# kngwyu/rogue-gym

Hardware: AMD Instinct MI355X
Metric: env-steps/sec (whole node) at 65 536 envs, 32x16 mini-dungeon (higher is better)
Workload: dtype u8/u16 integer state, f32 observation; 1 GPU; config-mini.json 32x16, 65536 envs per GPU (65536 total), gray-image obs [N,1,16,32] f32, max_steps 1000, auto-reset; envs_per_gpu=65536, parallelism=env-sharded x1, no data-path collective

## Files before the change

### rogue-gym_amd/csrc/rg_api.cpp

```cpp
#include <hip/hip_runtime.h>
#include <dlfcn.h>

#include <cstdio>
#include <cstdlib>
#include <cstring>
#include <mutex>
#include <random>
#include <string>
#include <vector>

#include "../../include/rogue_gym_hip.h"
#include "rg_state.h"
#include "rg_state_io.h"

extern "C" {
typedef struct ncclComm *ncclComm_t;
typedef struct { char internal[128]; } ncclUniqueId;
typedef int ncclResult_t;
typedef int ncclDataType_t;
}
static const ncclResult_t ncclSuccess = 0;
static const ncclDataType_t ncclUint8 = 1;

extern "C" {
// ... 2 lines not shown
void rgk_probe_clock(unsigned long long *out, int spin, hipStream_t st);
void rgk_regen(const RgState *SP, const RgConfig *c, int bulk, int spares, const uint32_t *mark, uint32_t target, uint32_t *err_any, hipStream_t st, hipEvent_t ev0, hipEvent_t ev1);
void rgk_regen_gate(const uint32_t *mark, uint32_t target, uint32_t *err_any, hipStream_t st);
void rgk_export(const RgState *S, uint32_t *err_any, void *o_screen, void *o_hist, void *o_status, void *o_flags, uint32_t *o_err, hipStream_t st);
int rgk_regen_lanes_supported(const RgConfig *c, int maze_cap);
int rgk_step_bound_capable(const RgConfig *c);
int rgk_regen_lanes(const RgState *SP, const RgConfig *c, uint32_t *q, int32_t *list, int bulk, int waves, int slots, hipStream_t st, hipEvent_t ev0, hipEvent_t ev1);
void rgk_debug_descend(const RgState *S, const RgConfig *c, hipStream_t st);
void rgk_render(const RgState *S, const RgConfig *c, hipStream_t st);
void rgk_encode(const uint8_t *screen, const uint8_t *hist, const int32_t *status, uint32_t *flags, uint32_t *err_any, int n, int hw, size_t rs, size_t rst,
                int symbols, int planes_sym, uint32_t sflag, int with_hist, int kind, float *out, const int32_t *ext, hipStream_t st);
void rgk_pack(const RgState *S, int with_hist, uint8_t *out, hipStream_t st);
void rgk_scatter_rows(const void *src, void *dst, const int32_t *ext, int n, int row_bytes, hipStream_t st);
void rgk_gather_keys(const uint8_t *keys, const int32_t *ext, uint8_t *dst, int n, hipStream_t st);
int rgk_obs(const RgState *S, const RgConfig *c, uint32_t sflag, int with_hist, int kind, float *out, uint32_t *err_any, int planes_sym, int bound, hipStream_t st, hipEvent_t ev0, hipEvent_t ev1);
int rgk_redraw(const RgState *S, const RgConfig *c, hipStream_t st);
int rgk_obs_typed(const RgState *S, const RgConfig *c, int kind, int dtype, uint32_t sflag, int with_hist, int planes_sym, void *out, uint32_t *err_any, hipStream_t st, hipEvent_t ev0,
                  hipEvent_t ev1);
int rgk_obs_crop(const RgState *S, const RgConfig *c, int kind, int ry, int rx, uint32_t sflag, int with_hist, int planes_sym, float *out, int32_t *centers,
                 uint32_t *err_any, hipStream_t st);
void rgk_state_save(const RgState *S, const RgIoLayout *L, const uint64_t *desc, const uint32_t *guard, const int32_t *ids, int k, uint8_t *out, hipStream_t st);
void rgk_state_load(const RgState *S, const RgIoLayout *L, const uint64_t *desc, const uint32_t *guard, const int32_t *ids, int k, const uint8_t *recs, uint32_t rec_bytes, uint8_t *ok,
                    uint8_t *mark, hipStream_t st);
}

#define RG_TIMED_KERNELS 5
struct rg_handle {
    RgParsed parsed;
    RgConfig cfg;
    RgState S;
// ... 5 lines not shown
    int lane_flip = 0;
    uint64_t lane_last = 0;
    uint8_t *pin_keys = nullptr;
    uint32_t *pin_err = nullptr;
    bool lane_regen = false;
    uint64_t step_count = 0;
    hipStream_t side = nullptr;
    int regen_idle_after = -1;
    int regen_bulk = 0;
    int device = 0;
    hipStream_t stream = nullptr;
    std::vector<void *> allocs;
    uint32_t *d_err = nullptr;
    uint8_t *d_keys = nullptr;
    bool render_pending = false;
    float *bound_out = nullptr; int bound_kind = 0; bool bound_valid = false;
    int32_t *obs_list_mem = nullptr; uint32_t *obs_cnt_mem = nullptr; float *gray_lut_mem = nullptr;
    int bound_steps = 0;
    int stair_gen = 0;
    float *obs_scratch = nullptr;
    size_t obs_scratch_cap = 0;
    std::vector<uint64_t> seed_lo, seed_hi;
    std::vector<uint8_t> reseed;
    std::vector<uint64_t> range_lo, range_span;
    unsigned long long *d_probe = nullptr;
    std::vector<rg_handle *> sub;
    std::vector<int> g_of, l_of;
    int32_t *d_ext = nullptr;
    std::vector<int32_t> ext;
    uint8_t *d_keys_sub = nullptr;
// ... 207 lines not shown
             dev_alloc(h, &P.p_exp, ns) && dev_alloc(h, &P.food, ns) && dev_alloc(h, &P.quiet, ns) && dev_alloc(h, &P.pack_gold, ns) && dev_alloc(h, &P.dlevel, ns) &&
             dev_alloc(h, &P.rng, 12 * ns) && dev_alloc(h, &P.room_rect, nr * ns) && dev_alloc(h, &P.room_meta, nr * ns) &&
             dev_alloc(h, &P.mon_w0, nr * ns) && dev_alloc(h, &P.mon_hp, nr * ns) && dev_alloc(h, &P.mon_exp, nr * ns) &&
             dev_alloc(h, &P.mon_cnt, ns) && dev_alloc(h, &P.gold_pos, nr * ns) && dev_alloc(h, &P.gold_amt, nr * ns) &&
             dev_alloc(h, &P.edge_a, ne * n) && dev_alloc(h, &P.edge_b, ne * n) && dev_alloc(h, &P.maze_stack, (size_t)maze_cap * n) &&
             dev_alloc(h, &P.on_stairs, ns);
        P.prof = nullptr;
        int lo = 0, hi = 0;
        if (ok && (hipDeviceGetStreamPriorityRange(&lo, &hi) != hipSuccess || hipStreamCreateWithPriority(&h->side, hipStreamNonBlocking, RG_DEV_ENV("ROGUE_GYM_HIP_SIDE_HIPRIO") ? hi : lo) != hipSuccess)) {
            h->err = "failed to create the background generation stream"; ok = false;
        }
        static const bool lanes_low = RG_DEV_ENV("ROGUE_GYM_HIP_LANES_LOWPRIO") != nullptr;
        if (ok && (hipStreamCreateWithPriority(&h->side2, hipStreamNonBlocking, lanes_low ? lo : (lo + hi) / 2) != hipSuccess || hipStreamCreateWithPriority(&h->side3, hipStreamNonBlocking, lanes_low ? lo : (lo + hi) / 2) != hipSuccess)) { h->err = "failed to create the background generation stream"; ok = false; }
    }
    ok = ok && dev_alloc(h, &h->d_SP, 1) && hipMemcpy(h->d_SP, &h->SP, sizeof(RgState), hipMemcpyHostToDevice) == hipSuccess;
    if (!ok) { g_create_err = h->err.empty() ? "device allocation failed" : h->err; destroy_handle(h); return 1; }
    if (hipMemset(S.screen, ' ', n * hw) != hipSuccess) { g_create_err = "hipMemset failed"; destroy_handle(h); return 1; }
    if (upload_seeds(h, n)) { g_create_err = h->err; destroy_handle(h); return 1; }
    h->S.stair_gen = h->stair_gen++;
    rgk_build(&h->S, &h->cfg, h->stream);
    hipError_t e = hipGetLastError();
    if (e == hipSuccess) e = hipStreamSynchronize(h->stream);
    if (e != hipSuccess) { g_create_err = std::string("k_build: ") + hipGetErrorString(e); destroy_handle(h); return 1; }
    h->render_pending = true;
    if (h->spares) {
        if (h->lane_regen && !(dev_alloc(h, &h->lane_q, 8) && dev_alloc(h, &h->lane_list, 2 * ns))) { g_create_err = h->err; destroy_handle(h); return 1; }
        if (h->lane_regen) (void)rgk_regen_lanes(&h->SP, &h->cfg, h->lane_q, h->lane_list, 1, 0, h->S.sp_slots, h->side2, nullptr, nullptr);
        else rgk_regen(&h->SP, &h->cfg, 1, 1, nullptr, 0, h->d_err, h->side, nullptr, nullptr);
        e = hipGetLastError();
        if (e == hipSuccess && !RG_DEV_ENV("ROGUE_GYM_HIP_ASYNC_FIRST_SPARES")) { e = hipStreamSynchronize(h->side); if (e == hipSuccess) e = hipStreamSynchronize(h->side2); if (e == hipSuccess) e = hipStreamSynchronize(h->side3); }
// ... 191 lines not shown
    if (!h->sub.empty()) {
        for (rg_handle *sh : h->sub) SUBCHK(h, sh, rg_reset(sh));
        h->screens_stale = true;
        return assemble_small(h);
    }
    h->S.stair_gen = h->stair_gen++;
    { TimedLaunch t(h, 3); rgk_build(&h->S, &h->cfg, h->stream); }
    HIPCHK(h, hipGetLastError());
    h->render_pending = true;
    h->bound_valid = false;
    return 0;
}

static int obs_common(rg_t *h, uint32_t status_flag, int with_hist, int kind, float *out_dev);
int rg_step(rg_t *h, const uint8_t *keys, int keys_on_device) { return rg_step_prefix(h, keys, h->S.n, keys_on_device); }
int rg_step_obs_gray(rg_t *h, const uint8_t *keys, int keys_on_device, uint32_t status_flag, int with_hist, float *out_dev) {
    return rg_step_prefix(h, keys, h->S.n, keys_on_device) ? 1 : obs_common(h, status_flag, with_hist, 0, out_dev);
}

int rg_step_prefix(rg_t *h, const uint8_t *keys, int n_keys, int keys_on_device) {
    HIPCHK(h, hipSetDevice(h->device));
    if (n_keys < 0) { h->err = "rg_step_prefix: negative key count"; return 1; }
    if (n_keys > h->S.n) n_keys = h->S.n;
    if (!h->sub.empty()) {
        const uint8_t *dkeys = keys;
        if (!keys_on_device) {
            if (!h->d_keys && !dev_alloc(h, &h->d_keys, (size_t)h->S.n)) return 1;
            HIPCHK(h, hipMemcpyAsync(h->d_keys, keys, (size_t)n_keys, hipMemcpyHostToDevice, h->stream));
            dkeys = h->d_keys;
        }
        for (rg_handle *sh : h->sub) {
            int m = 0;
            while (m < sh->S.n && sh->ext[m] < n_keys) m++;
            if (m) rgk_gather_keys(dkeys, sh->d_ext, sh->d_keys_sub, m, h->stream);
            SUBCHK(h, sh, rg_step_prefix(sh, sh->d_keys_sub, m, 1));
        }
        HIPCHK(h, hipGetLastError());
        h->screens_stale = true;
        return assemble_small(h);
    }
    if (flush_render(h)) return 1;
    const uint8_t *dk = keys;
    if (!keys_on_device) {
        HIPCHK(h, hipMemcpyAsync(h->d_keys, keys, (size_t)n_keys, hipMemcpyHostToDevice, h->stream));
        dk = h->d_keys;
    }
    h->S.n_keys = n_keys;
    static const int regen_every = RG_DEV_ENV("ROGUE_GYM_HIP_REGEN_EVERY") ? atoi(RG_DEV_ENV("ROGUE_GYM_HIP_REGEN_EVERY")) : 1;
    h->step_count++;
    bool regen = h->spares && (regen_every <= 1 || h->step_count % (uint64_t)regen_every == 0);
    if (regen && h->regen_idle_after >= 0) { if (h->regen_idle_after == 0) regen = false; else h->regen_idle_after--; }
    static const bool no_stair_waves = getenv("ROGUE_GYM_HIP_NO_STAIR_WAVES") != nullptr;
    {
        TimedLaunch t(h, 0, true);
        h->S.stair_gen = h->stair_gen++;
        h->S.obs_par = (int32_t)(h->step_count & 1); h->bound_steps++;
        (void)rgk_step(&h->S, h->d_SP, &h->cfg, dk, h->spares ? 1 : 0, no_stair_waves ? -1 : 0, h->stream, t.start_ev(), t.stop_ev());
    }
    HIPCHK(h, hipGetLastError());
    if (regen) {
        TimedLaunch t(h, 4, true);
        if (h->lane_regen) {
            static const int lane_waves = RG_DEV_ENV("ROGUE_GYM_HIP_LANE_WAVES") ? atoi(RG_DEV_ENV("ROGUE_GYM_HIP_LANE_WAVES")) : 256;
            static const int lane_every = RG_DEV_ENV("ROGUE_GYM_HIP_LANE_EVERY") ? atoi(RG_DEV_ENV("ROGUE_GYM_HIP_LANE_EVERY")) : 16;
            static const bool time_lanes = RG_DEV_ENV("ROGUE_GYM_HIP_TIME_LANES") != nullptr;
            const bool lanes_now = h->regen_bulk > 0 || h->step_count - h->lane_last >= (uint64_t)(lane_every > 0 ? lane_every : 1);
            static const int urgent_mode = RG_DEV_ENV("ROGUE_GYM_HIP_URGENT_AT0") ? 3 : 2;
            rgk_regen(&h->SP, &h->cfg, 0, urgent_mode, h->S.launch_mark, (uint32_t)h->S.stair_gen + 1u, h->d_err, h->side, time_lanes ? nullptr : t.start_ev(), time_lanes ? nullptr : t.stop_ev());
            if (time_lanes && !lanes_now) t.cancel();
            if (lanes_now) {
                h->lane_last = h->step_count;
                h->lane_flip ^= 1;
// ... 56 lines not shown
    HIPCHK(h, hipSetDevice(h->device));
    if (!h->sub.empty()) {
        for (rg_handle *sh : h->sub) {
            if (kind && sh->cfg.symbols > h->planes_sym) {
                h->err = "symbol image: a config of the batch has more symbols (" + std::to_string(sh->cfg.symbols) + ") than env 0's (" + std::to_string(h->planes_sym) +
                         "), which sets the channel count (python/src/lib.rs:281-285)";
                return 1;
            }
            SUBCHK(h, sh, obs_common(sh, status_flag, with_hist, kind, out_dev));
        }
        return 0;
    }
    {
        TimedLaunch t(h, 2, true);
        const bool bound = h->bound_out && out_dev == h->bound_out && kind == h->bound_kind && (status_flag & 0x1ffu) == 0 && !with_hist;
        if (rgk_obs(&h->S, &h->cfg, status_flag & 0x1ffu, with_hist ? 1 : 0, kind, out_dev, h->d_err, h->planes_sym, bound && h->S.obs_list && h->bound_valid && h->bound_steps == 1, h->stream, t.start_ev(), t.stop_ev())) {
            HIPCHK(h, hipGetLastError());
            h->render_pending = false;
            h->bound_valid = bound;
            h->bound_steps = 0;
            return 0;
        }
        t.cancel();
    }
    h->bound_valid = false;
    if (flush_render(h)) return 1;
    {
        TimedLaunch t(h, 2);
        rgk_encode(h->S.screen, h->S.hist, h->S.status, h->S.flags, h->d_err, h->S.n, h->S.hw, (size_t)h->S.hw, 10, h->cfg.symbols, h->planes_sym,
                   status_flag & 0x1ffu, with_hist ? 1 : 0, kind, out_dev, h->S.ext, h->stream);
    }
    HIPCHK(h, hipGetLastError());
// ... 846 lines not shown
```

### rogue-gym_amd/csrc/rg_kernels.hip

```cpp


#include "rg_device.h"


#include "rg_gen.h"


#ifdef RG_FINE_PROF
#define PFM(id) pf.mark(id)
#else
#define PFM(id) ((void)0)
#endif
struct Prof {
    unsigned long long *p; unsigned long long t, t0, r0; int k;
    __device__ __forceinline__ void start(unsigned long long *pp) { p = pp ? pp + (size_t)blockIdx.x * 64 : nullptr; k = 0; if (p) { r0 = __builtin_amdgcn_s_memrealtime(); t = t0 = __builtin_amdgcn_s_memtime(); } }
    __device__ __forceinline__ void rec(int phase, unsigned long long v) {
        if (p && threadIdx.x == 0 && k < 61) p[1 + k++] = ((unsigned long long)phase << 48) | (v & 0xffffffffffffull);
    }
    __device__ __forceinline__ void mark(int phase) {
        if (!p) return;
        unsigned long long now = __builtin_amdgcn_s_memtime();
        rec(phase, now - t);
        t = now;
    }
// ... 2088 lines not shown
#pragma nounroll
    for (int s0 = 0; s0 < nrooms; s0++)
        if ((actp >> (3 * s0)) & 2u) {
            const uint32_t m = mc[s0 * WAVE];
            const int x = POS_X(m), y = POS_Y(m);
            const uint32_t under = base_glyph(c, WV(w, WIN_K(x - w.ox, y - w.oy)), y);
            if ((under & 0x80u) && under != (0x80u | '*')) put(y * W + x, mt[(m >> 16) & 0xff]);
        }
    if (pl_moved && (base_glyph(c, WV(w, WIN_K(px - w.ox, py - w.oy)), py) & 0x80u)) put(py * W + px, '@');
    return true;
}

__device__ __forceinline__ void take_spares(const RgState &S, const RgState *__restrict__ SPd, const RgConfig &c, int lane, int e, bool taken, bool &on_stairs) {
    const uint64_t tm = __ballot(taken);
    if (!tm) return;
    const RgState &SP = *SPd;
    const int HW = S.hw, n = S.n, nrooms = c.room_num_x * c.room_num_y;
    const size_t ns = (size_t)n * S.sp_slots;
    int es = e;
    if (taken)
        for (int sl = S.sp_slots - 1; sl >= 0; sl--)
            if (__hip_atomic_load(&S.sp_ready[(size_t)sl * n + e], __ATOMIC_RELAXED, __HIP_MEMORY_SCOPE_AGENT) == 1u) es = sl * n + e;
    __builtin_amdgcn_fence(__ATOMIC_ACQUIRE, "agent");
    if ((HW & 7) == 0) {
        const int q = HW / 8;
        uint64_t mm = tm;
        while (mm) {
            const int s0 = __ffsll((long long)mm) - 1; mm &= mm - 1;
            const int s1 = mm ? __ffsll((long long)mm) - 1 : -1; if (mm) mm &= mm - 1;
            const int s2 = mm ? __ffsll((long long)mm) - 1 : -1; if (mm) mm &= mm - 1;
// ... 180 lines not shown
        uint64_t lag = __ballot(descends && ((old_flags & RG_FLAG_HIST_LAG) || ((old_flags & RG_FLAG_REDRAW) && (old_flags & RG_FLAG_HIST_STALE))));
        while (lag) {
            const int src = __ffsll((long long)lag) - 1;
            lag &= lag - 1;
            const int env_s = __shfl(e, src);
            const uint16_t *cp = S.cell + (size_t)env_s * S.hw;
            uint8_t *hp = S.hist + (size_t)env_s * S.hw;
            for (int i = lane; i < S.hw; i += WAVE) hp[i] = (cp[i] & C_VISITED) ? 1 : 0;
        }
    }
#pragma nounroll
    for (int pass = 0; pass < 2; ++pass) {
        pf.mark(1);
        if (pass == 1 && use_spares) {
            if (need_gen) {
                bool rdy = false;
                for (int sl = 0; sl < S.sp_slots; sl++) rdy = rdy || __hip_atomic_load(&S.sp_ready[(size_t)sl * S.n + e], __ATOMIC_RELAXED, __HIP_MEMORY_SCOPE_AGENT) == 1u;
                if (rdy) { taken = true; need_gen = false; n_taken++; }
            }
        }
        const bool regenerated = descends && pass == 0;
        if constexpr (BW == 1 || BW == 2) { if (pass == 0 && S.dc_walk) snapshot_walk_service(S, c, lane, e, descends); }
        const uint64_t nx_now = pass == 0 ? __ballot(need_gen && nxs == RG_NX_HIT) : 0ull;
        if (need_gen) n_inline++;
        gen_service<GM>(S, c, E, lane, e, need_gen, pass == 1, lds_grid, pf, nx_now);
        (void)regenerated;
        pf.mark(2);
        need_gen = false;
        if (pass == 1) break;

        bool running = live && act != ACT_NOOP;
        int iter = 0;
        while (__any(running)) {
// ... 116 lines not shown
    if (valid && err) {
        S.flags[et] = (old_flags & ~RG_FLAG_ERR_MASK) | err;
        S.reward[et] = 0.f;
        S.done[et] = (old_flags & RG_FLAG_TERMINAL) ? 1 : 0;
        atomicOr(S.err_any, err);
    } else if (valid && !live) {
        S.reward[et] = 0.f; S.done[et] = (old_flags & RG_FLAG_TERMINAL) ? 1 : 0;
    } else if (valid) {
        if (terminal && c.auto_reset) {
            if (taken) {
                E.dlevel = 1; E.gold = c.init_gold; E.hp = E.hpmax = c.init_hp; E.plvl = 1; E.exp = 0; E.food = c.hunger_time;
            }
            write_status(S, c, E);
            S.dc_len[et] = 0; S.dc_head[et] = 0; S.dc_part[et] = 0; S.dc_own[et] = 0;
            steps = 0;
            flags = RG_FLAG_REDRAW | RG_FLAG_HIST_DIRTY;
            klog_new_episode(S, et);
        }
        if (E.err) { flags |= E.err; atomicOr(S.err_any, E.err); }
        if (terminal) flags |= RG_FLAG_TERMINAL;
        if (!taken) store_env(S, E);
        S.steps[et] = steps;
        S.flags[et] = flags;
        S.done[et] = terminal ? 1 : 0;
        if (S.ovl && !taken && !inc_done && ((react & R_REDRAW) || descends || (terminal && c.auto_reset))) {
            for (int s0 = 0; s0 < nrooms_k; s0++) {
                const uint32_t mw = E.mc[s0 * WAVE];
                S.ovl[(size_t)s0 * S.n + et] = (uint16_t)(((mw >> 24) & MF_ALIVE) ? ((mw & 0xffffu) | OVL_UNKNOWN) : OVL_NONE);
            }
            S.ovl[(size_t)nrooms_k * S.n + et] = (uint16_t)(POS(E.px, E.py) | OVL_UNKNOWN);
        }
// ... 189 lines not shown
```

### rogue-gym_amd/csrc/rg_obs.hip

```cpp
#include <cstdlib>
#include "rg_device.h"

#define RENDER_THREADS 256
__device__ __forceinline__ bool in_same_room(const RgState &S, const RgConfig &c, int e, int ax, int ay, int bx, int by) {
    int id = room_id_of(c, ax, ay);
    if (id < 0 || room_id_of(c, bx, by) != id) return false;
    uint8_t meta = S.room_meta[id * S.n + e];
    if ((meta & RM_KIND_MASK) == RK_EMPTY) return true;
    int x0, y0, x1, y1;
    unpack_rect(S.room_rect[id * S.n + e], x0, y0, x1, y1);
    bool ina = ax >= x0 && ax < x1 && ay >= y0 && ay < y1, inb = bx >= x0 && bx < x1 && by >= y0 && by < y1;
    return ina == inb;
}

__global__ void __launch_bounds__(RENDER_THREADS) k_render(RgState S, RgConfig c) {
    __shared__ uint8_t s_scr[RG_MAX_W * RG_MAX_H];
    const int tid = threadIdx.x, W = c.width, H = c.height, HW = W * H, n = S.n;
    const int nrooms = c.room_num_x * c.room_num_y;
    for (int e = blockIdx.x; e < n; e += gridDim.x) {
        const uint32_t fl = S.flags[e];
        if (!(fl & RG_FLAG_REDRAW)) continue;
        const uint16_t *cell = S.cell + (size_t)e * HW;
        const bool upd_hist = !(fl & RG_FLAG_HIST_STALE);
        uint8_t *hist = S.hist + (size_t)e * HW;
// ... 344 lines not shown
            }
            if (KIND == 1 && bad) { atomicOr(&S.flags[e], RG_FLAG_ERR_TILE); atomicOr(err_any, RG_FLAG_ERR_TILE); }
            const uint32_t seen = BOUND ? RG_FLAG_SCR_CHANGED : 0u;
            if (redraw && lt == 0) {
                const uint32_t clr = seen | RG_FLAG_REDRAW | RG_FLAG_HIST_STALE | RG_FLAG_HIST_LAG | ((fl & RG_FLAG_HIST_STALE) ? 0u : RG_FLAG_HIST_DIRTY);
                const uint32_t set = (fl & RG_FLAG_HIST_STALE) ? RG_FLAG_HIST_LAG : 0u;
                if (KIND == 1) {
                    atomicAnd(&S.flags[e], ~clr);
                    if (set) atomicOr(&S.flags[e], set);
                } else S.flags[e] = (fl & ~clr) | set;
            } else if (BOUND && !redraw && lt == 0) atomicAnd(&S.flags[e], ~RG_FLAG_SCR_CHANGED);
        }
    }
}

#ifndef OBS_RUN
#define OBS_RUN 4
#endif
#ifndef OBS_STREAM_WAVES
#define OBS_STREAM_WAVES 16384
#endif
__global__ void __launch_bounds__(WAVE) k_obs_stream(RgState S, RgConfig c, float *__restrict__ out, int hi_prio) {
    if (hi_prio) __builtin_amdgcn_s_setprio(3);
    __shared__ float lutf[128];
    __shared__ uint8_t mtile[RG_MAX_ENEMY_KINDS + 6];
    __shared__ __align__(16) uint8_t scr[512];
    __shared__ ObsTabs tb;
    const int lane = threadIdx.x, W = c.width, HW = W * c.height, Q4 = HW >> 2, Q8 = HW >> 3, n = S.n;
    const int nrooms = c.room_num_x * c.room_num_y, rec_words = RG_OBS_REC_WORDS(nrooms);
    for (int g = lane; g < 128; g += WAVE) lutf[g] = (float)(uint8_t)tile_to_sym((uint32_t)g) / (float)(uint8_t)c.symbols;
    for (int g = lane; g < RG_MAX_ENEMY_KINDS + 6; g += WAVE) mtile[g] = c.mon[g].tile;
    lds_barrier();
    auto gray4 = [&](uint32_t w) {
        w &= 0x7f7f7f7fu;
        float4 v; v.x = lutf[w & 0xff]; v.y = lutf[(w >> 8) & 0xff]; v.z = lutf[(w >> 16) & 0xff]; v.w = lutf[w >> 24];
        return v;
    };
    struct Run { uint32_t fl, w0[OBS_RUN], w1[OBS_RUN]; };
    auto load_run = [&](int r, Run &R) {
        const int base = r * OBS_RUN, cnt = n - base;
        R.fl = lane < cnt && lane < OBS_RUN ? S.flags[base + lane] : 0u;
        const uint32_t *m = reinterpret_cast<const uint32_t *>(S.screen) + (size_t)base * Q4;
#pragma unroll
        for (int i = 0; i < OBS_RUN; i++) {
            R.w0[i] = i < cnt && lane < Q4 ? m[i * Q4 + lane] : 0u;
            R.w1[i] = i < cnt && lane + WAVE < Q4 ? m[i * Q4 + lane + WAVE] : 0u;
        }
    };
    const int nruns = (n + OBS_RUN - 1) / OBS_RUN;
    Run cur;
    load_run(blockIdx.x, cur);
    for (int r = blockIdx.x; r < nruns; r += gridDim.x) {
        const int base = r * OBS_RUN, cnt = n - base < OBS_RUN ? n - base : OBS_RUN;
        Run nxt;
        load_run(r + gridDim.x, nxt);
        const uint32_t fl = cur.fl;
#ifdef RG_EXP_OBS_STREAM_BOUND
        uint64_t rmask = 0;
#else
        uint64_t rmask = __ballot(fl & RG_FLAG_REDRAW);
#endif
        auto load_tiles = [&](int e, uint4 &v, uint32_t &rec) {
            v = lane < Q8 ? reinterpret_cast<const uint4 *>(S.cell + (size_t)e * HW)[lane] : make_uint4(0, 0, 0, 0);
            rec = lane < rec_words ? S.obs_rec[(size_t)e * rec_words + lane] : 0u;
        };
        uint4 tv = make_uint4(0, 0, 0, 0);
        uint32_t trec = 0;
        if (rmask) load_tiles(base + __builtin_ctzll(rmask), tv, trec);
        float4 *o = reinterpret_cast<float4 *>(out) + (size_t)base * Q4;
#pragma unroll
        for (int i = 0; i < OBS_RUN; i++) {
// ... 28 lines not shown
                    const uint32_t under = scr[y * W + x];
                    if (monster_shown(c, &tb, nrooms, px, py, x, y) && (under & 0x80u) && under != (0x80u | '*')) scr[y * W + x] = (uint8_t)(0x80u | mtile[(mw >> 16) & 0xff]);
                }
            }
            lds_barrier();
            if (lane == 0 && (scr[py * W + px] & 0x80u)) scr[py * W + px] = (uint8_t)(0x80u | '@');
            lds_barrier();
            uint32_t *m4 = reinterpret_cast<uint32_t *>(S.screen + (size_t)e * HW);
            float4 *oe = reinterpret_cast<float4 *>(out) + (size_t)e * Q4;
            for (int q = lane; q < Q4; q += WAVE) {
                const uint32_t g = reinterpret_cast<const uint32_t *>(scr)[q] & 0x7f7f7f7fu;
                m4[q] = g;
                store_obs(&oe[q], gray4(g));
            }
            if (lane == 0)
                S.flags[e] = (fle & ~(RG_FLAG_REDRAW | RG_FLAG_HIST_STALE | RG_FLAG_HIST_LAG | ((fle & RG_FLAG_HIST_STALE) ? 0u : RG_FLAG_HIST_DIRTY))) |
                             ((fle & RG_FLAG_HIST_STALE) ? RG_FLAG_HIST_LAG : 0u);
        }
        cur = nxt;
    }
}

#define RG_PUBLIC_FLAGS (RG_FLAG_TERMINAL | RG_FLAG_DEAD | RG_FLAG_MSG_MASK | RG_FLAG_ERR_MASK)
__global__ void __launch_bounds__(256) k_pack(const uint8_t *__restrict__ screen, const uint8_t *__restrict__ hist, const int32_t *__restrict__ status,
                                              const float *__restrict__ reward, const uint32_t *__restrict__ flags, int n, int hw, int with_hist, uint32_t *__restrict__ out) {
    const int qs = hw >> 2, qr = qs + 12 + (with_hist ? qs : 0);
    const size_t total = (size_t)n * qr;
    for (size_t g = (size_t)blockIdx.x * blockDim.x + threadIdx.x; g < total; g += (size_t)gridDim.x * blockDim.x) {
        const int e = (int)(g / qr), i = (int)(g - (size_t)e * qr);
        uint32_t v;
        if (i < qs) v = reinterpret_cast<const uint32_t *>(screen + (size_t)e * hw)[i];
// ... 391 lines not shown
    }
}

static void host_magic(RgCropArgs &a, int which, uint32_t d) {
    uint32_t l = 0;
    while ((1u << l) < d) l++;
    const uint32_t s = 30 + l;
    a.m[which] = (uint32_t)(((1ull << s) + d - 1) / d);
    a.shifts |= s << (6 * which);
}
extern "C" {
void rgk_render(const RgState *S, const RgConfig *c, hipStream_t st) {
    int blocks = S->n < 8192 ? S->n : 8192;
    hipLaunchKernelGGL(k_render, dim3(blocks), dim3(RENDER_THREADS), 0, st, *S, *c);
}
int rgk_obs(const RgState *S, const RgConfig *c, uint32_t sflag, int with_hist, int kind, float *out, uint32_t *err_any, int planes_sym, int bound, hipStream_t st, hipEvent_t ev0, hipEvent_t ev1) {
    int hw = c->width * c->height;
    if (hw & 7) return 0;
    if (c->room_num_x * c->room_num_y > RG_OBS_MAX_ROOMS || !S->obs_rec) return 0;
    int q8 = hw / 8;
    int tpe = q8 >= OBS_THREADS ? OBS_THREADS : ((q8 + 63) / 64) * 64;
    if (tpe > OBS_THREADS) tpe = OBS_THREADS;
    if (RG_OBS_REC_WORDS(c->room_num_x * c->room_num_y) > tpe) return 0;
    const int bthreads = tpe, epb = 1;
    const bool groups = S->ext != nullptr;
    size_t smem = 512 + 128 + 64 + (size_t)epb * OBS_ENV_BYTES(hw);
    int blocks = (S->n + epb - 1) / epb;
    {
        int cap = bthreads <= 64 ? 16384 : 8192;
#ifdef RG_DEV_KNOBS
        if (const char *ev = getenv("RG_OBS_BLOCKS")) cap = atoi(ev);
#endif
        if (blocks > cap) blocks = cap;
    }
    const int hi_prio = !(c->width <= 32 && c->room_num_x * c->room_num_y <= 32);
    bool stream = !kind && !groups && !bound && sflag == 0 && !with_hist && tpe == WAVE;
#ifdef RG_DEV_KNOBS
    if (const char *ev = getenv("RG_OBS_STREAM")) stream = stream && atoi(ev) != 0;
#endif
    if (stream) {
        int sblocks = (S->n + OBS_RUN - 1) / OBS_RUN, cap = OBS_STREAM_WAVES;
#ifdef RG_DEV_KNOBS
        if (const char *ev = getenv("RG_OBS_BLOCKS")) if (atoi(ev) > 0) cap = atoi(ev);
#endif
        if (sblocks > cap) sblocks = cap;
        if (ev0 || ev1) hipExtLaunchKernelGGL(k_obs_stream, dim3(sblocks), dim3(WAVE), 0, st, ev0, ev1, 0, *S, *c, out, hi_prio);
        else hipLaunchKernelGGL(k_obs_stream, dim3(sblocks), dim3(WAVE), 0, st, *S, *c, out, hi_prio);
        return 1;
    }
#define RG_LAUNCH_OBS(...) do { if (ev0 || ev1) hipExtLaunchKernelGGL((__VA_ARGS__), dim3(blocks), dim3(bthreads), (uint32_t)smem, st, ev0, ev1, 0, *S, *c, sflag, with_hist, out, err_any, tpe, epb, planes_sym, hi_prio); \
                               else hipLaunchKernelGGL((__VA_ARGS__), dim3(blocks), dim3(bthreads), smem, st, *S, *c, sflag, with_hist, out, err_any, tpe, epb, planes_sym, hi_prio); } while (0)
    if (bound && !groups && !kind) RG_LAUNCH_OBS(k_obs<0, false, true>);
    else if (bound && !groups) RG_LAUNCH_OBS(k_obs<1, false, true>);
    else if (!kind && !groups) RG_LAUNCH_OBS(k_obs<0, false>);
    else if (!kind) RG_LAUNCH_OBS(k_obs<0, true>);
    else if (!groups) RG_LAUNCH_OBS(k_obs<1, false>);
    else RG_LAUNCH_OBS(k_obs<1, true>);
#undef RG_LAUNCH_OBS
    return 1;
}
void rgk_encode(const uint8_t *screen, const uint8_t *hist, const int32_t *status, uint32_t *flags, uint32_t *err_any, int n, int hw, size_t rs, size_t rst,
                int symbols, int planes_sym, uint32_t sflag, int with_hist, int kind, float *out, const int32_t *ext, hipStream_t st) {
    if ((hw & 3) == 0 && (rs & 3) == 0) {
// ... 98 lines not shown
```

### rogue-gym_amd/csrc/rg_state.h

```cpp
#pragma once
#include <cstdint>

#include "rg_config.h"

#define C_SURF_MASK 0x0007u
#define C_DOOR      0x0008u
#define C_ATTR_SHIFT 4
#define C_VISITED   0x0010u
#define C_HIDDEN    0x0020u
#define C_VISIBLE   0x0040u
#define C_DRAWN     0x0080u
#define C_LOCKED    0x0100u
#define C_DARK      0x0200u
#define C_ATTR_MASK 0x03f0u
#define C_MAZE      0x0400u
#define C_GOLD      0x0800u

enum { S_PASSAGE = 0, S_FLOOR, S_WALLX, S_WALLY, S_STAIR, S_DOOR, S_TRAP, S_NONE };

#define RM_KIND_MASK 0x03u
#define RM_DARK      0x04u
#define RM_VISITED   0x08u
#define RM_HAS_GOLD  0x10u
enum { RK_NORMAL = 0, RK_MAZE = 1, RK_EMPTY = 2 };
// ... 12 lines not shown

#define RG_STAT_COLS 16
#define RG_NX_ASKED 1u
#define RG_NX_CLAIMED 6u
#define RG_NX_READY 3u
#define RG_NX_NONE 0u
#define RG_NX_DROP 4u
#define RG_NX_STALE 8u
#define RG_NX_HIT 9u
struct RgNext {
    uint16_t *cell;
    uint32_t *room_rect, *gold_pos, *gold_amt;
    uint8_t *room_meta;
    uint32_t *level;
};
struct RgState {
    int32_t n;
    int32_t hw;
    uint16_t *cell;
    uint8_t *screen;
    uint8_t *hist;
    uint16_t *p_pos;
    int32_t *p_hp, *p_hpmax, *p_lvl;
    uint32_t *p_exp, *food, *quiet, *pack_gold, *dlevel;
    uint32_t *steps, *flags;
    float *reward;
    uint8_t *done;
    uint32_t *rng;
    uint64_t *seed_lo, *seed_hi;
    uint8_t *reseed;
// ... 8 lines not shown
    uint32_t *mon_cnt;
    uint32_t *gold_pos, *gold_amt;
    uint32_t *edge_a, *edge_b;
    uint16_t *maze_stack;
    int32_t maze_cap;
    uint16_t *dc_map;
    uint16_t *dc_key;
    uint8_t *dc_head, *dc_len;
    uint16_t *dc_part, *dc_own;
    uint32_t *dc_walk;
    int keep_spares;
    int full_bfs;
    unsigned long long *prof;
    uint32_t *sp_ready;
    int32_t sp_slots;
    int32_t *status;
    uint32_t *obs_rec;
    uint16_t *ovl;
    float *bound_gray;
    const float *gray_lut;
    int32_t *obs_list;
    uint32_t *obs_cnt;
    int32_t obs_par;
    uint8_t *klog;
    uint32_t *klog_len;
    uint8_t *klog_cur;
    int32_t klog_cap;
    unsigned long long *stats;
    uint8_t *stair_mark;
    int32_t *stair_list;
// ... 13 lines not shown
```

Baseline: 757.1 million env-steps/s.

## Defer spare-level take from step kernel into streaming obs kernel

When a reset env picks up a pre-generated spare level, the step kernel now only records the chosen spare slot in the env flags instead of copying the spare state inline. The copy of cells, per-room words, player position and obs records is done by the streaming observation kernel before it renders, or by a standalone pending-take kernel when streaming obs isn't used. A host-built table of source/destination word pointers drives the copy. This takes the divergent bulk copy off the step kernel's critical path, at the cost of extra bookkeeping, a flags-bit encoding limited to a few slots, and a pre-pass over all runs in the obs kernel.

```diff
diff --git a/rogue-gym_amd/csrc/rg_api.cpp b/rogue-gym_amd/csrc/rg_api.cpp
--- a/rogue-gym_amd/csrc/rg_api.cpp
+++ b/rogue-gym_amd/csrc/rg_api.cpp
@@ -1,6 +1,7 @@
 #include <hip/hip_runtime.h>
 #include <dlfcn.h>
 
+#include <cstddef>
 #include <cstdio>
 #include <cstdlib>
 #include <cstring>
@@ -40,6 +41,8 @@
 void rgk_scatter_rows(const void *src, void *dst, const int32_t *ext, int n, int row_bytes, hipStream_t st);
 void rgk_gather_keys(const uint8_t *keys, const int32_t *ext, uint8_t *dst, int n, hipStream_t st);
 int rgk_obs(const RgState *S, const RgConfig *c, uint32_t sflag, int with_hist, int kind, float *out, uint32_t *err_any, int planes_sym, int bound, hipStream_t st, hipEvent_t ev0, hipEvent_t ev1);
+int rgk_obs_is_stream(const RgState *S, const RgConfig *c, uint32_t sflag, int with_hist, int kind, int bound);
+void rgk_take_pending(const RgState *S, const RgConfig *c, hipStream_t st);
 int rgk_redraw(const RgState *S, const RgConfig *c, hipStream_t st);
 int rgk_obs_typed(const RgState *S, const RgConfig *c, int kind, int dtype, uint32_t sflag, int with_hist, int planes_sym, void *out, uint32_t *err_any, hipStream_t st, hipEvent_t ev0,
                   hipEvent_t ev1);
@@ -75,6 +78,7 @@
     uint32_t *d_err = nullptr;
     uint8_t *d_keys = nullptr;
     bool render_pending = false;
+    bool take_pending = false;
     float *bound_out = nullptr; int bound_kind = 0; bool bound_valid = false;
     int32_t *obs_list_mem = nullptr; uint32_t *obs_cnt_mem = nullptr; float *gray_lut_mem = nullptr;
     int bound_steps = 0;
@@ -312,6 +316,36 @@
         if (ok && (hipStreamCreateWithPriority(&h->side2, hipStreamNonBlocking, lanes_low ? lo : (lo + hi) / 2) != hipSuccess || hipStreamCreateWithPriority(&h->side3, hipStreamNonBlocking, lanes_low ? lo : (lo + hi) / 2) != hipSuccess)) { h->err = "failed to create the background generation stream"; ok = false; }
     }
     ok = ok && dev_alloc(h, &h->d_SP, 1) && hipMemcpy(h->d_SP, &h->SP, sizeof(RgState), hipMemcpyHostToDevice) == hipSuccess;
+    if (ok && h->spares) {
+        const RgState &P = h->SP;
+        std::vector<RgTakeWord> tw;
+        auto word = [&](const uint32_t *src, uint32_t *dst, size_t src_off, size_t dst_off, uint32_t rec_word, uint32_t mon_slot) {
+            tw.push_back(RgTakeWord{(uint64_t)(uintptr_t)(src + src_off), (uint64_t)(uintptr_t)(dst + dst_off), rec_word | (mon_slot << 16), 0u});
+        };
+        const bool has_rec = S.obs_rec != nullptr;
+        for (size_t k = 0; k < 12; k++) word(P.rng, S.rng, k * ns, k * n, 0, 0);
+        word((const uint32_t *)P.p_hp, (uint32_t *)S.p_hp, 0, 0, 0, 0); word((const uint32_t *)P.p_hpmax, (uint32_t *)S.p_hpmax, 0, 0, 0, 0);
+        word((const uint32_t *)P.p_lvl, (uint32_t *)S.p_lvl, 0, 0, 0, 0);
+        word(P.p_exp, S.p_exp, 0, 0, 0, 0); word(P.food, S.food, 0, 0, 0, 0); word(P.quiet, S.quiet, 0, 0, 0, 0);
+        word(P.pack_gold, S.pack_gold, 0, 0, 0, 0); word(P.dlevel, S.dlevel, 0, 0, 0, 0); word(P.mon_cnt, S.mon_cnt, 0, 0, 0, 0);
+        for (size_t s = 0; s < nr; s++) {
+            word(P.mon_w0, S.mon_w0, s * ns, s * n, has_rec ? (uint32_t)(1 + s) : 0u, (uint32_t)(1 + s));
+            word(P.room_rect, S.room_rect, s * ns, s * n, has_rec ? (uint32_t)(1 + nr + 1 + s) : 0u, 0);
+            word((const uint32_t *)P.mon_hp, (uint32_t *)S.mon_hp, s * ns, s * n, 0, 0); word(P.mon_exp, S.mon_exp, s * ns, s * n, 0, 0);
+            word(P.gold_pos, S.gold_pos, s * ns, s * n, 0, 0); word(P.gold_amt, S.gold_amt, s * ns, s * n, 0, 0);
+        }
+        RgTakeTab hd;
+        memset(&hd, 0, sizeof hd);
+        hd.sp_cell = P.cell; hd.words = (int32_t)tw.size(); hd.sp_slots = S.sp_slots;
+        hd.sp_room_meta = P.room_meta; hd.sp_on_stairs = P.on_stairs; hd.sp_p_pos = P.p_pos; hd.room_meta = S.room_meta; hd.p_pos = S.p_pos;
+        hd.obs_rec = S.obs_rec; hd.ovl = S.ovl; hd.stair_mark = S.stair_mark; hd.stair_list = S.stair_list; hd.stair_cnt = S.stair_cnt; hd.sp_ready = S.sp_ready;
+        hd.reseed = S.reseed; hd.stats = S.stats; hd.keep_spares = S.keep_spares;
+        uint8_t *d_tab = nullptr;
+        ok = dev_alloc(h, &d_tab, offsetof(RgTakeTab, w) + tw.size() * sizeof(RgTakeWord)) &&
+             hipMemcpy(d_tab, &hd, offsetof(RgTakeTab, w), hipMemcpyHostToDevice) == hipSuccess &&
+             hipMemcpy(d_tab + offsetof(RgTakeTab, w), tw.data(), tw.size() * sizeof(RgTakeWord), hipMemcpyHostToDevice) == hipSuccess;
+        S.take_tab = reinterpret_cast<const RgTakeTab *>(d_tab);
+    }
     if (!ok) { g_create_err = h->err.empty() ? "device allocation failed" : h->err; destroy_handle(h); return 1; }
     if (hipMemset(S.screen, ' ', n * hw) != hipSuccess) { g_create_err = "hipMemset failed"; destroy_handle(h); return 1; }
     if (upload_seeds(h, n)) { g_create_err = h->err; destroy_handle(h); return 1; }
@@ -533,8 +567,33 @@
 
 static int obs_common(rg_t *h, uint32_t status_flag, int with_hist, int kind, float *out_dev);
 int rg_step(rg_t *h, const uint8_t *keys, int keys_on_device) { return rg_step_prefix(h, keys, h->S.n, keys_on_device); }
+static bool bound_pass(const rg_handle *h, uint32_t status_flag, int with_hist, int kind, const float *out_dev) {
+    const bool bound = h->bound_out && out_dev == h->bound_out && kind == h->bound_kind && (status_flag & 0x1ffu) == 0 && !with_hist;
+    return bound && h->S.obs_list && h->bound_valid && h->bound_steps == 1;
+}
 int rg_step_obs_gray(rg_t *h, const uint8_t *keys, int keys_on_device, uint32_t status_flag, int with_hist, float *out_dev) {
-    return rg_step_prefix(h, keys, h->S.n, keys_on_device) ? 1 : obs_common(h, status_flag, with_hist, 0, out_dev);
+    const bool can_defer = h->sub.empty() && !h->mixed && h->spares && h->S.take_tab && h->S.sp_slots <= (int)(RG_FLAG_TAKE_MASK >> RG_FLAG_TAKE_SHIFT);
+    bool defer = can_defer && !h->S.obs_list && !h->bound_out && rgk_obs_is_stream(&h->S, &h->cfg, status_flag & 0x1ffu, with_hist ? 1 : 0, 0, 0);
+    bool standalone = false;
+#ifdef RG_DEV_KNOBS
+    if (const char *ev = getenv("RG_TAKE_DEFER")) defer = atoi(ev) == 2 ? can_defer : (defer && atoi(ev) != 0);
+    if (const char *ev = getenv("RG_TAKE_STANDALONE")) standalone = atoi(ev) != 0;
+#endif
+    h->S.defer_take = defer ? 1 : 0;
+    int rc = rg_step_prefix(h, keys, h->S.n, keys_on_device);
+    h->S.defer_take = 0;
+    if (!rc && h->take_pending && (standalone || !rgk_obs_is_stream(&h->S, &h->cfg, status_flag & 0x1ffu, with_hist ? 1 : 0, 0, bound_pass(h, status_flag, with_hist, 0, out_dev)))) {
+        rgk_take_pending(&h->S, &h->cfg, h->stream);
+        h->take_pending = false;
+    }
+    if (!rc) rc = obs_common(h, status_flag, with_hist, 0, out_dev);
+    if (h->take_pending) {
+        (void)hipSetDevice(h->device);
+        rgk_take_pending(&h->S, &h->cfg, h->stream);
+        h->take_pending = false;
+        if (hipGetLastError() != hipSuccess && !rc) { h->err = "k_take_pending: launch failed"; rc = 1; }
+    }
+    return rc;
 }
 
 int rg_step_prefix(rg_t *h, const uint8_t *keys, int n_keys, int keys_on_device) {
@@ -558,6 +617,9 @@
         h->screens_stale = true;
         return assemble_small(h);
     }
+#ifdef RG_DEV_KNOBS
+    if (h->take_pending) { fprintf(stderr, "rogue_gym_hip: a deferred spare take was left pending across a C-ABI call\n"); abort(); }
+#endif
     if (flush_render(h)) return 1;
     const uint8_t *dk = keys;
     if (!keys_on_device) {
@@ -575,6 +637,7 @@
         h->S.stair_gen = h->stair_gen++;
         h->S.obs_par = (int32_t)(h->step_count & 1); h->bound_steps++;
         (void)rgk_step(&h->S, h->d_SP, &h->cfg, dk, h->spares ? 1 : 0, no_stair_waves ? -1 : 0, h->stream, t.start_ev(), t.stop_ev());
+        if (h->S.defer_take) h->take_pending = true;
     }
     HIPCHK(h, hipGetLastError());
     if (regen) {
@@ -661,8 +724,9 @@
     {
         TimedLaunch t(h, 2, true);
         const bool bound = h->bound_out && out_dev == h->bound_out && kind == h->bound_kind && (status_flag & 0x1ffu) == 0 && !with_hist;
-        if (rgk_obs(&h->S, &h->cfg, status_flag & 0x1ffu, with_hist ? 1 : 0, kind, out_dev, h->d_err, h->planes_sym, bound && h->S.obs_list && h->bound_valid && h->bound_steps == 1, h->stream, t.start_ev(), t.stop_ev())) {
+        if (const int launched = rgk_obs(&h->S, &h->cfg, status_flag & 0x1ffu, with_hist ? 1 : 0, kind, out_dev, h->d_err, h->planes_sym, bound_pass(h, status_flag, with_hist, kind, out_dev), h->stream, t.start_ev(), t.stop_ev())) {
             HIPCHK(h, hipGetLastError());
+            if (launched == 2) h->take_pending = false;
             h->render_pending = false;
             h->bound_valid = bound;
             h->bound_steps = 0;
diff --git a/rogue-gym_amd/csrc/rg_kernels.hip b/rogue-gym_amd/csrc/rg_kernels.hip
--- a/rogue-gym_amd/csrc/rg_kernels.hip
+++ b/rogue-gym_amd/csrc/rg_kernels.hip
@@ -2126,6 +2126,7 @@
 __device__ __forceinline__ void take_spares(const RgState &S, const RgState *__restrict__ SPd, const RgConfig &c, int lane, int e, bool taken, bool &on_stairs) {
     const uint64_t tm = __ballot(taken);
     if (!tm) return;
+    if (S.defer_take) { if (taken) on_stairs = false; return; }
     const RgState &SP = *SPd;
     const int HW = S.hw, n = S.n, nrooms = c.room_num_x * c.room_num_y;
     const size_t ns = (size_t)n * S.sp_slots;
@@ -2336,9 +2337,13 @@
         pf.mark(1);
         if (pass == 1 && use_spares) {
             if (need_gen) {
-                bool rdy = false;
-                for (int sl = 0; sl < S.sp_slots; sl++) rdy = rdy || __hip_atomic_load(&S.sp_ready[(size_t)sl * S.n + e], __ATOMIC_RELAXED, __HIP_MEMORY_SCOPE_AGENT) == 1u;
-                if (rdy) { taken = true; need_gen = false; n_taken++; }
+                int slot = -1;
+                for (int sl = S.sp_slots - 1; sl >= 0; sl--)
+                    if (__hip_atomic_load(&S.sp_ready[(size_t)sl * S.n + e], __ATOMIC_RELAXED, __HIP_MEMORY_SCOPE_AGENT) == 1u) slot = sl;
+                if (slot >= 0) {
+                    taken = true; need_gen = false; n_taken++;
+                    if (S.defer_take) flags |= (uint32_t)(slot + 1) << RG_FLAG_TAKE_SHIFT;
+                }
             }
         }
         const bool regenerated = descends && pass == 0;
@@ -2485,7 +2490,7 @@
             write_status(S, c, E);
             S.dc_len[et] = 0; S.dc_head[et] = 0; S.dc_part[et] = 0; S.dc_own[et] = 0;
             steps = 0;
-            flags = RG_FLAG_REDRAW | RG_FLAG_HIST_DIRTY;
+            flags = RG_FLAG_REDRAW | RG_FLAG_HIST_DIRTY | (flags & RG_FLAG_TAKE_MASK);
             klog_new_episode(S, et);
         }
         if (E.err) { flags |= E.err; atomicOr(S.err_any, E.err); }
diff --git a/rogue-gym_amd/csrc/rg_obs.hip b/rogue-gym_amd/csrc/rg_obs.hip
--- a/rogue-gym_amd/csrc/rg_obs.hip
+++ b/rogue-gym_amd/csrc/rg_obs.hip
@@ -382,6 +382,75 @@
     }
 }
 
+__device__ __forceinline__ void take_words(const RgTakeTab *__restrict__ T, int stair_gen, int n, int lane, int e, int es, int nrooms) {
+    typedef __attribute__((address_space(1))) uint32_t g32;
+    const int nw = T->words;
+    uint32_t *rec = T->obs_rec + (size_t)e * RG_OBS_REC_WORDS(nrooms);
+    uint16_t *ovl = T->ovl;
+    for (int j = lane; j < nw; j += WAVE) {
+        const RgTakeWord d = T->w[j];
+        const uint32_t v = *(const g32 *)(d.src + ((uint64_t)(uint32_t)es << 2));
+        *(g32 *)(d.dst + ((uint64_t)(uint32_t)e << 2)) = v;
+        const uint32_t ri = d.meta & 0xffffu, mon = d.meta >> 16;
+        if (ri) rec[ri - 1] = v;
+        if (mon && ovl) ovl[(size_t)(mon - 1) * n + e] = (uint16_t)(((v >> 24) & MF_ALIVE) ? ((v & 0xffffu) | 0x40u) : 0xffffu);
+    }
+    const size_t ns = (size_t)n * T->sp_slots;
+    for (int s = lane; s < nrooms; s += WAVE) {
+        const uint8_t m = T->sp_room_meta[s * ns + es];
+        T->room_meta[(size_t)s * n + e] = m;
+        if (T->obs_rec) reinterpret_cast<uint8_t *>(&rec[2 * nrooms + 1])[s] = m;
+    }
+    if (lane == WAVE - 1) {
+        const uint32_t pp = T->sp_p_pos[es];
+        const bool on = T->sp_on_stairs[es] != 0;
+        T->p_pos[e] = (uint16_t)pp;
+        if (T->obs_rec) rec[nrooms] = pp;
+        if (ovl) ovl[(size_t)nrooms * n + e] = (uint16_t)(pp | 0x40u);
+        if (on) {
+            const int w = (stair_gen + 1) & 1;
+            T->stair_mark[(size_t)w * n + e] = 1;
+            T->stair_list[(size_t)w * n + atomicAdd(&T->stair_cnt[(stair_gen + 1) % 3], 1u)] = e;
+        }
+    }
+}
+__device__ __forceinline__ void take_done(const RgTakeTab *__restrict__ T, int lane, int e, int es, int dev_col) {
+    const bool keep = T->keep_spares && T->reseed[e] == 0;
+    asm volatile("s_waitcnt vmcnt(0)" ::: "memory");
+    if (lane == 0 && !keep) __hip_atomic_store(&T->sp_ready[es], 0u, __ATOMIC_RELAXED, __HIP_MEMORY_SCOPE_AGENT);
+#ifdef RG_DEV_KNOBS
+    if (lane == 0 && T->stats) atomicAdd(&T->stats[dev_col], 1ull);
+#else
+    (void)dev_col;
+#endif
+}
+__device__ __forceinline__ void take_wave(const RgTakeTab *__restrict__ T, uint16_t *__restrict__ cell, uint32_t *__restrict__ flags, int stair_gen, int n, int HW, int nrooms,
+                                          int lane, int e0, uint32_t fl, int dev_col) {
+    uint64_t pm = __ballot(fl & RG_FLAG_TAKE_MASK);
+    asm volatile("" : "+v"(T));
+    __builtin_amdgcn_fence(__ATOMIC_ACQUIRE, "agent");
+    while (pm) {
+        const int i = __builtin_ctzll(pm);
+        pm &= pm - 1;
+        const int e = e0 + i;
+        const uint32_t fle = __builtin_amdgcn_readlane(fl, i);
+        const int es = (int)(((fle & RG_FLAG_TAKE_MASK) >> RG_FLAG_TAKE_SHIFT) - 1u) * n + e;
+        const uint16_t *sp = T->sp_cell + (size_t)es * HW;
+        uint16_t *dp = cell + (size_t)e * HW;
+        if ((HW & 7) == 0) for (int q = lane; q < (HW >> 3); q += WAVE) reinterpret_cast<uint4 *>(dp)[q] = reinterpret_cast<const uint4 *>(sp)[q];
+        else for (int q = lane; q < HW; q += WAVE) dp[q] = sp[q];
+        take_words(T, stair_gen, n, lane, e, es, nrooms);
+        if (lane == 0) flags[e] = fle & ~RG_FLAG_TAKE_MASK;
+        take_done(T, lane, e, es, dev_col);
+    }
+}
+__global__ void __launch_bounds__(WAVE) k_take_pending(RgState S, RgConfig c) {
+    const int lane = threadIdx.x, e0 = blockIdx.x * WAVE;
+    const uint32_t fl = e0 + lane < S.n ? S.flags[e0 + lane] : 0u;
+    if (!__ballot(fl & RG_FLAG_TAKE_MASK)) return;
+    take_wave(S.take_tab, S.cell, S.flags, S.stair_gen, S.n, S.hw, c.room_num_x * c.room_num_y, lane, e0, fl, 10);
+}
+
 #ifndef OBS_RUN
 #define OBS_RUN 4
 #endif
@@ -396,9 +465,6 @@
     __shared__ ObsTabs tb;
     const int lane = threadIdx.x, W = c.width, HW = W * c.height, Q4 = HW >> 2, Q8 = HW >> 3, n = S.n;
     const int nrooms = c.room_num_x * c.room_num_y, rec_words = RG_OBS_REC_WORDS(nrooms);
-    for (int g = lane; g < 128; g += WAVE) lutf[g] = (float)(uint8_t)tile_to_sym((uint32_t)g) / (float)(uint8_t)c.symbols;
-    for (int g = lane; g < RG_MAX_ENEMY_KINDS + 6; g += WAVE) mtile[g] = c.mon[g].tile;
-    lds_barrier();
     auto gray4 = [&](uint32_t w) {
         w &= 0x7f7f7f7fu;
         float4 v; v.x = lutf[w & 0xff]; v.y = lutf[(w >> 8) & 0xff]; v.z = lutf[(w >> 16) & 0xff]; v.w = lutf[w >> 24];
@@ -418,11 +484,20 @@
     const int nruns = (n + OBS_RUN - 1) / OBS_RUN;
     Run cur;
     load_run(blockIdx.x, cur);
+    if (__ballot(cur.fl & RG_FLAG_TAKE_MASK)) take_wave(S.take_tab, S.cell, S.flags, S.stair_gen, n, HW, nrooms, lane, blockIdx.x * OBS_RUN, cur.fl, 9);
+    for (int r = blockIdx.x + gridDim.x; r < nruns; r += gridDim.x) {
+        const int base = r * OBS_RUN;
+        const uint32_t fl = lane < n - base && lane < OBS_RUN ? S.flags[base + lane] : 0u;
+        if (__ballot(fl & RG_FLAG_TAKE_MASK)) take_wave(S.take_tab, S.cell, S.flags, S.stair_gen, n, HW, nrooms, lane, base, fl, 9);
+    }
+    for (int g = lane; g < 128; g += WAVE) lutf[g] = (float)(uint8_t)tile_to_sym((uint32_t)g) / (float)(uint8_t)c.symbols;
+    for (int g = lane; g < RG_MAX_ENEMY_KINDS + 6; g += WAVE) mtile[g] = c.mon[g].tile;
+    lds_barrier();
     for (int r = blockIdx.x; r < nruns; r += gridDim.x) {
         const int base = r * OBS_RUN, cnt = n - base < OBS_RUN ? n - base : OBS_RUN;
+        const uint32_t fl = cur.fl;
         Run nxt;
         load_run(r + gridDim.x, nxt);
-        const uint32_t fl = cur.fl;
 #ifdef RG_EXP_OBS_STREAM_BOUND
         uint64_t rmask = 0;
 #else
@@ -481,7 +556,7 @@
                 store_obs(&oe[q], gray4(g));
             }
             if (lane == 0)
-                S.flags[e] = (fle & ~(RG_FLAG_REDRAW | RG_FLAG_HIST_STALE | RG_FLAG_HIST_LAG | ((fle & RG_FLAG_HIST_STALE) ? 0u : RG_FLAG_HIST_DIRTY))) |
+                S.flags[e] = (fle & ~(RG_FLAG_TAKE_MASK | RG_FLAG_REDRAW | RG_FLAG_HIST_STALE | RG_FLAG_HIST_LAG | ((fle & RG_FLAG_HIST_STALE) ? 0u : RG_FLAG_HIST_DIRTY))) |
                              ((fle & RG_FLAG_HIST_STALE) ? RG_FLAG_HIST_LAG : 0u);
         }
         cur = nxt;
@@ -903,6 +978,20 @@
     int blocks = S->n < 8192 ? S->n : 8192;
     hipLaunchKernelGGL(k_render, dim3(blocks), dim3(RENDER_THREADS), 0, st, *S, *c);
 }
+int rgk_obs_is_stream(const RgState *S, const RgConfig *c, uint32_t sflag, int with_hist, int kind, int bound) {
+    const int hw = c->width * c->height, nr = c->room_num_x * c->room_num_y;
+    if ((hw & 7) || nr > RG_OBS_MAX_ROOMS || !S->obs_rec) return 0;
+    const int tpe = hw / 8 >= OBS_THREADS ? OBS_THREADS : ((hw / 8 + 63) / 64) * 64;
+    if (RG_OBS_REC_WORDS(nr) > tpe) return 0;
+    bool stream = !kind && !S->ext && !bound && sflag == 0 && !with_hist && tpe == WAVE;
+#ifdef RG_DEV_KNOBS
+    if (const char *ev = getenv("RG_OBS_STREAM")) stream = stream && atoi(ev) != 0;
+#endif
+    return stream ? 1 : 0;
+}
+void rgk_take_pending(const RgState *S, const RgConfig *c, hipStream_t st) {
+    hipLaunchKernelGGL(k_take_pending, dim3((S->n + WAVE - 1) / WAVE), dim3(WAVE), 0, st, *S, *c);
+}
 int rgk_obs(const RgState *S, const RgConfig *c, uint32_t sflag, int with_hist, int kind, float *out, uint32_t *err_any, int planes_sym, int bound, hipStream_t st, hipEvent_t ev0, hipEvent_t ev1) {
     int hw = c->width * c->height;
     if (hw & 7) return 0;
@@ -923,11 +1012,7 @@
         if (blocks > cap) blocks = cap;
     }
     const int hi_prio = !(c->width <= 32 && c->room_num_x * c->room_num_y <= 32);
-    bool stream = !kind && !groups && !bound && sflag == 0 && !with_hist && tpe == WAVE;
-#ifdef RG_DEV_KNOBS
-    if (const char *ev = getenv("RG_OBS_STREAM")) stream = stream && atoi(ev) != 0;
-#endif
-    if (stream) {
+    if (rgk_obs_is_stream(S, c, sflag, with_hist, kind, bound)) {
         int sblocks = (S->n + OBS_RUN - 1) / OBS_RUN, cap = OBS_STREAM_WAVES;
 #ifdef RG_DEV_KNOBS
         if (const char *ev = getenv("RG_OBS_BLOCKS")) if (atoi(ev) > 0) cap = atoi(ev);
@@ -935,7 +1020,7 @@
         if (sblocks > cap) sblocks = cap;
         if (ev0 || ev1) hipExtLaunchKernelGGL(k_obs_stream, dim3(sblocks), dim3(WAVE), 0, st, ev0, ev1, 0, *S, *c, out, hi_prio);
         else hipLaunchKernelGGL(k_obs_stream, dim3(sblocks), dim3(WAVE), 0, st, *S, *c, out, hi_prio);
-        return 1;
+        return 2;
     }
 #define RG_LAUNCH_OBS(...) do { if (ev0 || ev1) hipExtLaunchKernelGGL((__VA_ARGS__), dim3(blocks), dim3(bthreads), (uint32_t)smem, st, ev0, ev1, 0, *S, *c, sflag, with_hist, out, err_any, tpe, epb, planes_sym, hi_prio); \
                                else hipLaunchKernelGGL((__VA_ARGS__), dim3(blocks), dim3(bthreads), smem, st, *S, *c, sflag, with_hist, out, err_any, tpe, epb, planes_sym, hi_prio); } while (0)
diff --git a/rogue-gym_amd/csrc/rg_state.h b/rogue-gym_amd/csrc/rg_state.h
--- a/rogue-gym_amd/csrc/rg_state.h
+++ b/rogue-gym_amd/csrc/rg_state.h
@@ -50,6 +50,19 @@
     uint8_t *room_meta;
     uint32_t *level;
 };
+#define RG_FLAG_TAKE_SHIFT 24
+#define RG_FLAG_TAKE_MASK  0x07000000u
+struct RgTakeWord { uint64_t src, dst; uint32_t meta, pad; };
+struct RgTakeTab {
+    const uint16_t *sp_cell;
+    const uint8_t *sp_room_meta, *sp_on_stairs; const uint16_t *sp_p_pos;
+    uint8_t *room_meta; uint16_t *p_pos;
+    uint32_t *obs_rec; uint16_t *ovl; uint8_t *stair_mark; int32_t *stair_list; uint32_t *stair_cnt; uint32_t *sp_ready; const uint8_t *reseed;
+    unsigned long long *stats;
+    int32_t keep_spares, sp_slots, words, pad;
+    RgTakeWord w[1];
+};
+
 struct RgState {
     int32_t n;
     int32_t hw;
@@ -88,6 +101,8 @@
     unsigned long long *prof;
     uint32_t *sp_ready;
     int32_t sp_slots;
+    int32_t defer_take;
+    const RgTakeTab *take_tab;
     int32_t *status;
     uint32_t *obs_rec;
     uint16_t *ovl;
```

Measured after the change: 727.8 million env-steps/s. -3.9%, worse.
